# ishine/minimax-speech

Hardware: AMD Instinct MI355X
Metric: 24 kHz audio-seconds generated per wall-second per node (CosyVoice2-0.5B-shaped LM + flow + DAC-VAE, end to end) (higher is better)
Workload: dtype bf16

## Files before the change

include/mmx_hip.h:

```cpp
#ifndef MMX_HIP_H
#define MMX_HIP_H
#include <stdint.h>
#ifdef __cplusplus
extern "C" {
#endif

#ifndef __HIP__
typedef struct ihipStream_t* hipStream_t;
#endif

#define MMX_F32 0
#define MMX_BF16 1
#define MMX_X2 2
#define MMX_X3 3
#define MMX_X2W 0x12
#define MMX_X3W 0x13
#define MMX_H2 4
#define MMX_H2W 0x14

#define MMX_ACT_NONE 0
#define MMX_ACT_LRELU 1
#define MMX_ACT_GELU 2
#define MMX_ACT_SILU 3
#define MMX_ACT_MISH 4
#define MMX_ACT_TANH 5

int mmx_abi_version(void);

typedef struct MmxGemmParams {
    const void* A;
    const void* W;
    const float* bias;
    const float* residual;
    const float* rowmask;
    const float* alpha;
    float* out_f32;
    void* out_act;
    int64_t lda, ldw, ldr, ldo_f, ldo_a;
    int64_t a_bstride, w_bstride, r_bstride, rm_bstride, of_bstride, oa_bstride;
    int64_t row_off, row_lo, row_hi;
// ... 92 lines not shown

int mmx_decode_prep(const float* x, int64_t ldx, int B, int K, const float* gamma, float* h, int64_t ldh, void* xs,
                    float* ssq, int dtype, hipStream_t stream);
int mmx_skinny2(const void* xs, int B, int K, int N, const void* wp, const float* bias, const float* ssq_in, float eps,
                int epi, float* out, int64_t ldo, void* xs_out, const float* gamma_next, float* ssq_out,
                int tiles_per_wg, int ksplit, float* part, int64_t part_floats, int32_t* tickets, int dtype,
                hipStream_t stream);

int mmx_rope_kv_store(const float* qkv, int64_t ldqkv, int64_t qkv_bs, int B, int rows, int Hq, int Hkv, int D,
                      const float* inv_freq, const int32_t* pos, void* q_out, int64_t ldq, int64_t q_bs,
                      void* kc, void* vc, const int32_t* block_table, int max_pages, int page,
                      int dtype, hipStream_t stream);
int mmx_paged_attn(const void* q, int64_t ldq, int64_t q_bs, int B, int rows, int Hq, int Hkv, int D, float scale,
                   const int32_t* pos, const void* kc, const void* vc, const int32_t* block_table, int max_pages,
                   int page, void* out, int64_t ldo, int64_t o_bs, int dtype, hipStream_t stream);
#define MMX_DA_PACKED 1
#define MMX_DA_PER_HEAD 2
#define MMX_DA_SPLIT 4
#define MMX_DA_H2 8
#define MMX_DA_ONE_HEAD 16
int mmx_decode_attn(const float* qkv, int64_t ldqkv, int B, int Hq, int Hkv, int D, const float* inv_freq,
                    const float* rope_tab, const int32_t* pos, void* kc, void* vc, const int32_t* block_table, int max_pages, int page,
                    float scale, void* out, int64_t ldo, int dtype, int out_packed, hipStream_t stream);
int mmx_decode_attn_fin(const float* qkv, int64_t ldqkv, int B, int Hq, int Hkv, int D, const float* inv_freq,
                        const float* rope_tab, const int32_t* pos, const int32_t* finished, void* kc, void* vc,
                        const int32_t* block_table, int max_pages, int page, float scale, void* out, int64_t ldo, int dtype,
                        int out_packed, hipStream_t stream);
int mmx_swiglu(const float* gu, int64_t ldgu, int rows, int I, void* out, int64_t ldo, int dtype, hipStream_t stream);

int mmx_sample_step(const float* logits, int64_t ldl, int V, int B, int eos_id, int top_k, float top_p,
// ... 134 lines not shown
```

minimax-speech_amd/csrc/common.h:

```cpp
#pragma once
#include <hip/hip_runtime.h>
#include <stdint.h>
#include "../../include/mmx_hip.h"

#ifndef MMX_LAB
#define MMX_LAB 0
#endif
constexpr bool LAB = MMX_LAB != 0;

#define MMX_OK 0
#define MMX_EARG (-1)
#define MMX_CHECK_ARG(c) do { if (!(c)) return MMX_EARG; } while (0)
#define MMX_LAUNCH_CHECK() do { hipError_t e_ = hipGetLastError(); if (e_ != hipSuccess) return -(int)e_ - 1000; } while (0)

#define MMX_ACT_DTYPE(d) ((d) >= 2 ? 0 : (d))

#define MMX_LDS_OPT_IN(fn, bytes)                                                                                   \
    do {                                                                                                            \
        if ((bytes) > 64 * 1024) {                                                                                  \
            static bool done_[64] = {};                                                                             \
            int dev_ = 0;                                                                                           \
            if (hipGetDevice(&dev_) != hipSuccess || dev_ < 0 || dev_ >= 64) return MMX_EARG;                       \
            if (!done_[dev_]) {                                                                                     \
                hipError_t e_ = hipFuncSetAttribute((const void*)(fn), hipFuncAttributeMaxDynamicSharedMemorySize, 160 * 1024); \
// ... 55 lines not shown
#pragma unroll
    for (int o = 32; o > 0; o >>= 1) v += __shfl_xor(v, o, 64);
    return v;
}
__device__ __forceinline__ float wave_max(float v) {
#pragma unroll
    for (int o = 32; o > 0; o >>= 1) v = fmaxf(v, __shfl_xor(v, o, 64));
    return v;
}
__device__ __forceinline__ double wave_sum_f64(double v) {
#pragma unroll
    for (int o = 32; o > 0; o >>= 1) v += __shfl_xor(v, o, 64);
    return v;
}

enum { ACT_NONE = 0, ACT_LRELU = 1, ACT_GELU = 2, ACT_SILU = 3, ACT_MISH = 4, ACT_TANH = 5 };

__device__ __forceinline__ float erf_fast(float x) {
    const float ax = fabsf(x);
    const float t = __builtin_amdgcn_rcpf(1.0f + 0.3275911f * ax);
    float p = 1.061405429f;
    p = p * t - 1.453152027f;
    p = p * t + 1.421413741f;
    p = p * t - 0.284496736f;
    p = p * t + 0.254829592f;
    const float r = 1.0f - p * t * __expf(-ax * ax);
    return copysignf(r, x);
}

typedef float f32x2_t __attribute__((ext_vector_type(2)));
__device__ __forceinline__ f32x2_t gelu_fast2(f32x2_t v) {
// ... 90 lines not shown
```

minimax-speech_amd/csrc/gemm.hip:

```cpp
#include <algorithm>
#include "common.h"
#include "gemm.h"
#include <utility>

template <typename T> struct Frag;
template <> struct Frag<bf16_t> {
    static constexpr int CH = 8;
    static constexpr int LDS_ROW = 48;
};
template <> struct Frag<float> {
    static constexpr int CH = 4;
    static constexpr int LDS_ROW = 40;
};

template <typename T, typename TA, int NS, int BM, int BN, int WM, int WN, int NWP = 1>
__global__ __launch_bounds__(256) void gemm_win_kernel(GemmParams p) {
    constexpr int BK = 32;
    constexpr bool XS = NS > 1;
    static_assert(NWP == 1 || NWP == NS, "weight planes: as many as activation planes");
    static_assert(!XS || (sizeof(T) == 2 && sizeof(TA) == 4), "split build: bf16 weights, fp32 activations");
    static_assert(XS || sizeof(T) == sizeof(TA), "one storage type otherwise");
    constexpr int CH = Frag<T>::CH;
    constexpr int CPR = BK / CH;
    constexpr int CHA = 16 / sizeof(TA);
    constexpr int CPRA = BK / CHA;
    constexpr int LR = Frag<T>::LDS_ROW;
    constexpr int MF = BM / WM / 16, NF = BN / WN / 16;
    constexpr int A_CHUNKS = (BM * CPRA + 255) / 256, W_CHUNKS = (BN * CPR + 255) / 256;
    constexpr bool A_FULL = (BM * CPRA) % 256 == 0, W_FULL = (BN * CPR) % 256 == 0;
    constexpr bool PRECISE = sizeof(TA) == 4;
// ... 169 lines not shown
            load_tile(kt + STAGES, sc);
            __syncthreads();
            compute(decltype(sc)::value & 1);
        });
    }
    for_each_slot([&](auto sc) {
        const int kt = kt0 + decltype(sc)::value;
        if (kt < nk) {
            store_tile(decltype(sc)::value & 1, sc);
            __syncthreads();
            compute(decltype(sc)::value & 1);
        }
    });

    __syncthreads();
    constexpr int WNC = BN / WN;
    constexpr int CW = WNC / 4;
    constexpr int LDC = WNC + 4;
    float* Cs = reinterpret_cast<float*>(smem) + wave * 16 * LDC;
    float* outf = p.out_f32 ? p.out_f32 + (long)b * p.of_bstride : nullptr;
    TA* outa = p.out_act ? reinterpret_cast<TA*>(p.out_act) + (long)b * p.oa_bstride : nullptr;
    const float* res = p.residual ? p.residual + (long)b * p.r_bstride : nullptr;
    const float* rmask = p.rowmask ? p.rowmask + (long)b * p.rm_bstride : nullptr;
    constexpr int VA = 16 / sizeof(TA);
    const bool vec_f = outf && (p.ldo_f % 4 == 0) && (p.out_off % 4 == 0) && (p.of_bstride % 4 == 0) && ((uintptr_t)p.out_f32 % 16 == 0);
    const bool vec_a = outa && (p.ldo_a % VA == 0) && (p.out_off % VA == 0) && (p.oa_bstride % VA == 0) && ((uintptr_t)p.out_act % 16 == 0) && (CW % VA == 0);
    const bool vec_r = res && (p.ldr % 4 == 0) && (p.r_bstride % 4 == 0) && ((uintptr_t)p.residual % 16 == 0);
    const int erow = lane >> 2, ecol = (lane & 3) * CW;
    auto epilogue = [&](auto act_k, auto act2_k) {
    constexpr int ACT = decltype(act_k)::value, ACT2 = decltype(act2_k)::value;
// ... 92 lines not shown
    }
    };
    using std::integral_constant;
    switch (p.act) {
        case ACT_LRELU: epilogue(integral_constant<int, ACT_LRELU>{}, integral_constant<int, ACT_NONE>{}); break;
        case ACT_GELU: epilogue(integral_constant<int, ACT_GELU>{}, integral_constant<int, ACT_NONE>{}); break;
        case ACT_SILU: epilogue(integral_constant<int, ACT_SILU>{}, integral_constant<int, ACT_NONE>{}); break;
        case ACT_MISH: epilogue(integral_constant<int, ACT_MISH>{}, integral_constant<int, ACT_NONE>{}); break;
        case ACT_TANH: epilogue(integral_constant<int, ACT_TANH>{}, integral_constant<int, ACT_NONE>{}); break;
        default:
            if (p.act2 == ACT_MISH) epilogue(integral_constant<int, ACT_NONE>{}, integral_constant<int, ACT_MISH>{});
            else epilogue(integral_constant<int, ACT_NONE>{}, integral_constant<int, ACT_NONE>{});
    }
}

template <typename T, typename TA, int NS, int BM, int BN, int WM, int WN, int NWP = 1>
static int launch_cfg(const GemmParams& p, hipStream_t s) {
    dim3 grid((p.N + BN - 1) / BN, (p.M + BM - 1) / BM, p.batch);
    size_t lds = (size_t)2 * (NS * BM + NWP * BN) * Frag<T>::LDS_ROW * sizeof(T);
    const size_t lds_epi = (size_t)4 * 16 * (BN / WN + 4) * sizeof(float);
    if (lds_epi > lds) lds = lds_epi;
    MMX_LDS_OPT_IN((gemm_win_kernel<T, TA, NS, BM, BN, WM, WN, NWP>), lds);
    hipLaunchKernelGGL((gemm_win_kernel<T, TA, NS, BM, BN, WM, WN, NWP>), grid, dim3(256), lds, s, p);
    MMX_LAUNCH_CHECK();
    return MMX_OK;
}

template <typename T, typename TA, int NS, int NWP = 1>
static int launch_T(const GemmParams& p, hipStream_t s, int force_tile) {
    constexpr int CH = Frag<T>::CH;
    constexpr int CHA = 16 / sizeof(TA);
    MMX_CHECK_ARG(p.A && p.W && p.M > 0 && p.N > 0 && p.batch > 0 && p.ntaps >= 1);
    MMX_CHECK_ARG(p.cin % CH == 0 && p.lda % CHA == 0 && p.ldw % CH == 0);
    MMX_CHECK_ARG(p.a_bstride % CHA == 0 && p.w_bstride % CH == 0);
    MMX_CHECK_ARG(p.ldw % NWP == 0 && (p.ldw / NWP) % CH == 0 && p.ldw / NWP >= ((p.ntaps * p.cin + 31) / 32) * 32);
    MMX_CHECK_ARG(p.bias_mod > 0 && p.alpha_mod > 0 && p.row_stride >= 1);
    MMX_CHECK_ARG(((uintptr_t)p.A % 16) == 0 && ((uintptr_t)p.W % 16) == 0);
    MMX_CHECK_ARG(p.out_f32 || p.out_act);
    const long a_rows = std::min<long>(p.row_hi, (long)(p.M - 1) * p.row_stride + (long)(p.ntaps - 1) * p.dil + p.row_off + 1);
    MMX_CHECK_ARG((double)a_rows * (double)p.lda * sizeof(TA) < 2147483000.0 &&
                  (double)p.N * (double)p.ldw * sizeof(T) < 2147483000.0);
    MMX_CHECK_ARG(p.act2 == ACT_NONE || (p.act2 == ACT_MISH && p.act == ACT_NONE));
    auto blocks = [&](int bm, int bn) { return (long)((p.M + bm - 1) / bm) * ((p.N + bn - 1) / bn) * p.batch; };
    if constexpr (NWP > 1) {
        if (force_tile != 0 && force_tile != MMX_TILE_64x64 && force_tile != MMX_TILE_32x64) return MMX_EARG;
        if (force_tile != MMX_TILE_32x64 && (force_tile == MMX_TILE_64x64 || blocks(64, 64) >= 64 || p.M > 32))
            return launch_cfg<T, TA, NS, 64, 64, 2, 2, NWP>(p, s);
        return launch_cfg<T, TA, NS, 32, 64, 1, 4, NWP>(p, s);
    }
    switch (force_tile) {
        case 0: break;
        case MMX_TILE_128x128: return launch_cfg<T, TA, NS, 128, 128, 2, 2>(p, s);
        case MMX_TILE_128x64: return launch_cfg<T, TA, NS, 128, 64, 4, 1>(p, s);
        case MMX_TILE_64x64: return launch_cfg<T, TA, NS, 64, 64, 2, 2>(p, s);
        case MMX_TILE_32x64: return launch_cfg<T, TA, NS, 32, 64, 1, 4>(p, s);
        default: return MMX_EARG;
    }
// ... 21 lines not shown
```

minimax-speech_amd/csrc/llm.hip:

```cpp
#include "act_layout.h"
#include <type_traits>

template <typename T>
__global__ void pack_skinny_kernel(const T* __restrict__ w, long ldw, int N, int K, const float* __restrict__ kscale,
                                   int half, T* __restrict__ wp) {
    constexpr int E = sizeof(T) == 2 ? 8 : 4;
    constexpr int KB = E * 4;
    const long total = (long)((N + 15) / 16) * (K / KB) * 64 * E;
    for (long idx = (long)blockIdx.x * blockDim.x + threadIdx.x; idx < total; idx += (long)gridDim.x * blockDim.x) {
        int j = idx % E;
        long t = idx / E;
        int lane = t % 64;
        t /= 64;
        int kb = t % (K / KB);
        int tile = t / (K / KB);
        int col = lane & 15, g = lane >> 4;
        int row;
        if (half > 0) row = (tile & 1) * half + (tile >> 1) * 16 + col;
        else row = tile * 16 + col;
        int kk = kb * KB + g * E + j;
        float v = 0.f;
        if (row < N && (half == 0 || ((tile >> 1) * 16 + col) < half)) {
            v = Cvt<T>::to_f(w[(long)row * ldw + kk]);
            if (kscale) v *= kscale[kk];
// ... 418 lines not shown
    }
}
extern "C" int mmx_paged_attn(const void* q, int64_t ldq, int64_t q_bs, int B, int rows, int Hq, int Hkv, int D, float scale,
                              const int32_t* pos, const void* kc, const void* vc, const int32_t* block_table, int max_pages,
                              int page, void* out, int64_t ldo, int64_t o_bs, int dtype, hipStream_t stream) {
    dtype = MMX_ACT_DTYPE(dtype);
    MMX_CHECK_ARG(q && pos && kc && vc && block_table && out && B > 0 && rows > 0 && D == 64 && Hq % Hkv == 0 && page > 0);
    const size_t max_ctx = (size_t)max_pages * page;
    size_t lds = (64 + 8 + 4 * 64 + max_ctx) * 4;
    MMX_CHECK_ARG(lds <= 160 * 1024);
    return dispatch_dtype(dtype, [&](auto el) {
        using T = decltype(el);
        MMX_LDS_OPT_IN(paged_attn_kernel<T>, lds);
        hipLaunchKernelGGL(paged_attn_kernel<T>, dim3(Hq, rows, B), dim3(256), lds, stream, (const T*)q, ldq, q_bs, Hq, Hkv, scale, pos, (const T*)kc,
                           (const T*)vc, block_table, max_pages, page, (T*)out, ldo, o_bs);
        return launch_status();
    });
}

template <typename T>
struct Raw8 {
    uint4 a, b;
    __device__ __forceinline__ void load(const T* p) {
        a = *reinterpret_cast<const uint4*>(p);
        if constexpr (sizeof(T) == 4) b = *reinterpret_cast<const uint4*>(p + 4);
    }
    __device__ __forceinline__ void to_float(float o[8]) const {
        const unsigned w[4] = {a.x, a.y, a.z, a.w};
        if constexpr (sizeof(T) == 2) {
#pragma unroll
// ... 419 lines not shown
```

minimax-speech_amd/mmx/_lib.py:

```python
import ctypes as C
import os

import torch

F32, BF16 = 0, 1
X2, X3 = 2, 3
X2W, X3W = 0x12, 0x13
H2, H2W = 4, 0x14
DA_PACKED, DA_PER_HEAD, DA_SPLIT, DA_H2, DA_ONE_HEAD = 1, 2, 4, 8, 16
ACT = {"none": 0, "lrelu": 1, "gelu": 2, "silu": 3, "mish": 4, "tanh": 5}
TORCH_DT = {F32: torch.float32, BF16: torch.bfloat16, X2: torch.float32, X3: torch.float32, X2W: torch.float32, X3W: torch.float32}
WEIGHT_DT = {F32: torch.float32, BF16: torch.bfloat16, X2: torch.bfloat16, X3: torch.bfloat16, X2W: torch.bfloat16, X3W: torch.bfloat16}
ESIZE = {F32: 4, BF16: 2, X2: 4, X3: 4}
WPLANES = {X2W: 2, X3W: 3}
DTYPE_NAMES = {"f32": F32, "bf16": BF16, "x": X2, "x2": X2, "x3": X3}


def is_split(dtype):
    return dtype in (X2, X3, X2W, X3W)

_HERE = os.path.dirname(os.path.abspath(__file__))
LIB_PATH = os.environ.get("MMX_LIB") or os.path.join(os.path.dirname(_HERE), "lib", "libmmx_hip.so")

SYMBOLS = [
    "mmx_abi_version", "mmx_gemm_win", "mmx_gemm_win_tile", "mmx_rownorm", "mmx_groupnorm", "mmx_act_rows", "mmx_gather_rows", "mmx_copy2d", "mmx_est_pack",
    "mmx_sinusoidal_emb", "mmx_cfg_euler", "mmx_attn_dense", "mmx_attn_flash_bf16", "mmx_attn_flash_fp8", "mmx_attn_relpos_bf16", "mmx_attn_relpos_x", "mmx_attn_flash_x", "mmx_attn_flash_xs", "mmx_conv_cout1_tanh", "mmx_conv_cin1", "mmx_vae_sample", "mmx_resample_linear", "mmx_prefetch4", "mmx_mask_rows",
    "mmx_est_tail", "mmx_est_resnet", "mmx_dac_ru", "mmx_pack_skinny", "mmx_skinny_gemm", "mmx_skinny2", "mmx_decode_prep", "mmx_rope_kv_store", "mmx_paged_attn", "mmx_decode_attn", "mmx_decode_attn_fin", "mmx_swiglu", "mmx_sample_step",
    "mmx_sample_step_tab", "mmx_logmel", "mmx_pool_rows", "mmx_logmel_w", "mmx_s3_rope_fsmn", "mmx_fsq_encode", "mmx_resample_sinc", "mmx_kweight_blocks", "mmx_loudness_gate", "mmx_scale_rows",
    "mmx_spec_dist", "mmx_wave_sums", "mmx_gate_threshold", "mmx_gate_analyze", "mmx_gate_synthesize",
    "mmx_stoi_select", "mmx_stoi_bands", "mmx_stoi_score",
]


class GemmParams(C.Structure):
    _fields_ = [
        ("A", C.c_void_p), ("W", C.c_void_p), ("bias", C.c_void_p), ("residual", C.c_void_p),
        ("rowmask", C.c_void_p), ("alpha", C.c_void_p), ("out_f32", C.c_void_p), ("out_act", C.c_void_p),
        ("lda", C.c_int64), ("ldw", C.c_int64), ("ldr", C.c_int64), ("ldo_f", C.c_int64), ("ldo_a", C.c_int64),
        ("a_bstride", C.c_int64), ("w_bstride", C.c_int64), ("r_bstride", C.c_int64), ("rm_bstride", C.c_int64),
        ("of_bstride", C.c_int64), ("oa_bstride", C.c_int64),
        ("row_off", C.c_int64), ("row_lo", C.c_int64), ("row_hi", C.c_int64),
        ("out_off", C.c_int64), ("out_len", C.c_int64),
# ... 115 lines not shown
```

minimax-speech_amd/mmx/llm.py:

```python
import math
from typing import Dict, List, Optional

import torch

from . import ops
from ._lib import BF16, F32, H2, TORCH_DT, WEIGHT_DT, X3, X3W, is_split
from .flow import Graphed

ST_POS, ST_STEP, ST_NOUT, ST_FIN, ST_MINLEN, ST_MAXLEN, ST_SEQ, ST_ERR = range(8)


class PageAllocator:

    def __init__(self, n_pages: int):
        self.free_pages = list(range(n_pages - 1, -1, -1))
        self.n_pages = n_pages

    @property
    def n_free(self) -> int:
        return len(self.free_pages)

    def alloc(self, n: int) -> List[int]:
        if n > len(self.free_pages):
            raise RuntimeError(f"KV cache exhausted: {n} pages wanted, {len(self.free_pages)} free of {self.n_pages}")
# ... 26 lines not shown
            pk = lambda w, g=None, ih=0: ops.pack_skinny(c(w), dtype=dt, kscale=ks(g), interleave_half=ih)
        self.n_layers = len({k.split(".")[4] for k in sd if k.startswith(prefix + ".layers.")})
        self.H = sd[prefix + ".norm.weight"].shape[0]
        self.I = sd[prefix + ".layers.0.mlp.gate_proj.weight"].shape[0]
        self.layers, self.pf_layers = [], []
        for l in range(self.n_layers):
            p = f"{prefix}.layers.{l}"
            a = p + ".self_attn"
            wqkv = torch.cat([f(a + ".q_proj.weight"), f(a + ".k_proj.weight"), f(a + ".v_proj.weight")], 0)
            bqkv = torch.cat([f(a + ".q_proj.bias"), f(a + ".k_proj.bias"), f(a + ".v_proj.bias")], 0).contiguous()
            wgu = torch.cat([f(p + ".mlp.gate_proj.weight"), f(p + ".mlp.up_proj.weight")], 0)
            g1, g2 = f(p + ".input_layernorm.weight"), f(p + ".post_attention_layernorm.weight")
            if gemm_packs:
                self.pf_layers.append(dict(
                    wqkv=ops.pack_linear(c(wqkv), dt), wo=ops.pack_linear(c(f(a + ".o_proj.weight")), dt),
                    wgu=ops.pack_linear(c(wgu), dt), wdown=ops.pack_linear(c(f(p + ".mlp.down_proj.weight")), dt), g1=g1, g2=g2))
            self.layers.append(dict(wqkv=pk(wqkv, g1), bqkv=bqkv, wo=pk(f(a + ".o_proj.weight")), wgu=pk(wgu, g2, self.I),
                                    wdown=pk(f(p + ".mlp.down_proj.weight")), g1=g1, g2=g2))
            del wqkv, wgu
        self.norm_w = f(prefix + ".norm.weight")
        self.embed_tokens = f(prefix + ".embed_tokens.weight")
        if "llm_decoder.weight" in sd:
            self.wdec = pk(f("llm_decoder.weight"), self.norm_w)
            self.bdec = f("llm_decoder.bias")
            self.speech_emb = f("speech_embedding.weight")
            self.llm_emb = f("llm_embedding.weight")
        else:
            self.wdec = self.bdec = self.speech_emb = self.llm_emb = None
        self.inv_freq = (1.0 / (rope_theta ** (torch.arange(0, head_dim, 2, dtype=torch.int64).float() / head_dim))).to(self.dev)
        self.max_pages = (max_ctx + page - 1) // page
        self.max_out = self.max_pages * page
        ang = torch.arange(self.max_out, dtype=torch.float32)[:, None] * self.inv_freq.cpu()[None, :]
        self.rope_tab = torch.cat([ang.cos(), ang.sin()], dim=1).contiguous().to(self.dev)
        npages = max_batch * self.max_pages if kv_pages is None else int(kv_pages)
        self.trash_page = npages
        self.kc = torch.zeros(self.n_layers, npages + 1, kv_heads, page, head_dim, dtype=self.tdt, device=self.dev)
        self.vc = torch.zeros_like(self.kc)
        self.pages = PageAllocator(npages)


class LlmEngine:
    gqa_min_batch = 1 << 30
    use_v2 = True
    lm_planes = "f16x2"
    prefetch = 0
    skip_finished = True

    def __init__(self, sd: Dict[str, torch.Tensor], dtype=BF16, device="cuda", max_batch=1, max_ctx=2048, page=16,
                 heads=14, kv_heads=2, head_dim=64, rope_theta=1e6, eps=1e-6, speech_token_size=6561, use_graphs=True,
                 prefix="llm.model.model", share_from=None, kv_pages=None, wplanes=False, lm_planes=None, decode_on=None,
                 prompt_on=None):
        if share_from is not None:
            m, v2 = share_from.model, share_from.v2 if decode_on is None else decode_on == "planes"
            dtype, h2, wplanes, gemm_packs = m.dtype, m.h2, m.wplanes, bool(m.pf_layers)
        else:
            wplanes = dtype == X3 and ops.resolve_wplanes(wplanes, (v for k, v in sd.items() if v.dim() >= 2 and ("proj" in k or k == "llm_decoder.weight")))
            planes = lm_planes or self.lm_planes
            if planes not in ("f16x2", "bf16x3"):
                raise ValueError(f"lm_planes {planes!r}: 'f16x2' or 'bf16x3'")
            v2, gemm_packs = self.use_v2 if decode_on is None else decode_on == "planes", True
            h2 = dtype == X3 and planes == "f16x2" and v2
# ... 280 lines not shown
            for b, x in enumerate(lm_inputs):
                self._prefill(x, 0, b, head=True)
                self.state[ST_POS, b] = x.shape[0] - 1
        self._tail(B)
        self._fresh_decode_graph()

    def _prefill_batch(self, lm_inputs):
        B, H = self.B, self.H
        Ls = [int(x.shape[0]) for x in lm_inputs]
        Lm = max(Ls)
        R = B * Lm
        h = torch.zeros(B, Lm, H, device=self.dev)
        for b, x in enumerate(lm_inputs):
            h[b, :Ls[b]].copy_(x)
        h = h.reshape(R, H)
        self._gemm_layers(h, B, Lm, torch.zeros(B, dtype=torch.int32, device=self.dev), self.block_table)
        last = torch.tensor([b * Lm + Ls[b] - 1 for b in range(B)], dtype=torch.long, device=self.dev)
        hl = h.index_select(0, last)
        self.h[:B].copy_(hl)
        self.h_act[:B].copy_(hl)
        self.state[ST_POS].copy_(torch.tensor([L - 1 for L in Ls], dtype=torch.int32))

    def _gemm_layers(self, h, B, Lm, pos, block_table):
        m = self.model
        dt, H, I = m.dtype, m.H, m.I
        R = B * Lm
        a = torch.empty(R, H, dtype=m.tdt, device=self.dev)
        qkv = torch.empty(R, (m.Hq + 2 * m.Hkv) * m.D, device=self.dev)
        q = torch.empty(R, m.Hq * m.D, dtype=m.tdt, device=self.dev)
        att = torch.empty(R, m.Hq * m.D, dtype=m.tdt, device=self.dev)
        gu = torch.empty(R, 2 * I, device=self.dev)
        act = torch.empty(R, I, dtype=m.tdt, device=self.dev)
        for l, (w, ws) in enumerate(zip(m.pf_layers, m.layers)):
            ops.rownorm(h, w["g1"], None, m.eps, rows=R, C_=H, rms=True, out_act=a, dtype=dt)
            ops.linear(a, w["wqkv"], H, dtype=dt, bias=ws["bqkv"], out_f32=qkv)
            ops.rope_kv_store(qkv, m.inv_freq, pos, q, m.kc[l], m.vc[l], block_table, B=B, rows=Lm,
                              Hq=m.Hq, Hkv=m.Hkv, page=m.page, dtype=dt)
            ops.paged_attn(q, pos, m.kc[l], m.vc[l], block_table, att, B=B, rows=Lm, Hq=m.Hq,
                           Hkv=m.Hkv, page=m.page, dtype=dt)
            ops.linear(att, w["wo"], m.Hq * m.D, dtype=dt, residual=h, out_f32=h)
            ops.rownorm(h, w["g2"], None, m.eps, rows=R, C_=H, rms=True, out_act=a, dtype=dt)
            ops.linear(a, w["wgu"], H, dtype=dt, out_f32=gu)
            ops.swiglu(gu, act, rows=R, I=I, dtype=dt)
            ops.linear(act, w["wdown"], I, dtype=dt, residual=h, out_f32=h)

    def _prefill(self, x, pos0, slot, head=False, norm_out=None):
        m = self.model
        x = x.to(self.dev, torch.float32).contiguous()
        for c0 in range(0, x.shape[0], 64):
            hc, hca = self._prefill_chunk(x[c0:c0 + 64], pos0 + c0, slot)
            if norm_out is not None:
                ops.rownorm(hc, m.norm_w, None, m.eps, rows=hc.shape[0], C_=m.H, rms=True, out_f32=norm_out[c0:c0 + 64], dtype=F32)
        if head:
            self.h[slot].copy_(hc[-1])
            self.h_act[slot].copy_(hca[-1])

    def _prefill_chunk(self, xc, pos0, b):
        rows = xc.shape[0]
        if self.prompt_on == "gemm":
            hc = xc.to(self.dev, torch.float32).clone()
            self._gemm_layers(hc, 1, rows, torch.tensor([pos0], dtype=torch.int32, device=self.dev), self.block_table[b:b + 1].contiguous())
            return hc, hc.to(self.tdt)
        if not hasattr(self, "_pf"):
            self._pf = dict(h=torch.zeros(64, self.H, device=self.dev), ha=torch.zeros(64, self.H, dtype=self.tdt, device=self.dev),
                            pos=torch.zeros(1, dtype=torch.int32, device=self.dev),
                            bt=torch.zeros(1, self.max_pages, dtype=torch.int32, device=self.dev), graphs={})
        pf = self._pf
        pf["h"][:rows].copy_(xc)
        pf["ha"][:rows].copy_(xc)
        pf["pos"].fill_(pos0)
        pf["bt"].copy_(self.block_table[b:b + 1])
        if rows not in pf["graphs"]:
            pf["graphs"][rows] = Graphed(lambda r=rows: self._layers(pf["h"][:r], pf["ha"][:r], 1, r, pf["pos"], pf["bt"]), self.use_graphs)
        pf["graphs"][rows]()
        return pf["h"][:rows], pf["ha"][:rows]

# ... 183 lines not shown
```

minimax-speech_amd/mmx/ops.py:

```python
import ctypes as C
import math

import torch

from . import _lib as L
from ._lib import ACT, BF16, F32, check, i64, load, stream, _p


def round_up(x, m):
    return (x + m - 1) // m * m


class Planed(torch.Tensor):
    """A packed weight held as bf16 PLANES hi + [mid +] lo = w of an fp32 checkpoint's values (include/mmx_hip.h MMX_X2W / MMX_X3W).
    The type is the marker: gemm() / skinny2() switch to the weight-plane dtype code when they are handed one; views and row
    slices keep the type (torch's default __torch_function__)."""


def weight_planes(w: torch.Tensor, n: int):
    out, r = [], w.float()
    for _ in range(n):
        t = r.to(torch.bfloat16)
        out.append(t)
        r = r - t.float()
# ... 66 lines not shown
                      row_hi=(row_hi if row_hi is not None else (1 << 40)), out_off=out_off,
                      out_len=(out_len if out_len is not None else (1 << 62)), M=M, N=N, batch=batch,
                      ntaps=ntaps, cin=cin, dil=dil, bias_mod=(bias_mod or N), alpha_mod=(alpha_mod or N),
                      bias_per_row=int(bias_per_row), act=ACT[act], act2=ACT[act2], slope=slope, row_stride=row_stride)
    L.gemm_win(p, dtype, tile)


def linear(x, Wp, K, *, dtype, bias=None, act="none", act2="none", residual=None, rowmask=None, out_f32=None,
           out_act=None):
    N = Wp.shape[0]
    M = x.numel() // x.shape[-1]
    gemm(x, Wp, M, N, dtype=dtype, lda=x.shape[-1], cin=K, bias=bias, act=act, act2=act2,
         residual=residual, ldr=N, rowmask=rowmask, out_f32=out_f32, ldo_f=N, out_act=out_act, ldo_a=N)


def conv1d(x, Wp, *, T, Cin, k, dtype, dil=1, pad_left=0, batch=1, bias=None, act="none", slope=0.1, residual=None,
           rowmask=None, alpha=None, out_f32=None, out_act=None, T_out=None, act2="none", stride=1):
    Cout = Wp.shape[0]
    T_out = T if T_out is None else T_out
    gemm(x, Wp, T_out, Cout, dtype=dtype, lda=Cin, cin=Cin, ntaps=k, dil=dil, row_off=-pad_left, row_lo=0, row_hi=T, row_stride=stride,
         batch=batch, a_bstride=T * Cin, bias=bias, act=act, act2=act2, slope=slope,
         residual=residual, ldr=Cout, r_bstride=T_out * Cout, rowmask=rowmask, rm_bstride=T_out,
         alpha=alpha, out_f32=out_f32, ldo_f=Cout, of_bstride=T_out * Cout,
         out_act=out_act, ldo_a=Cout, oa_bstride=T_out * Cout)


def convtranspose1d(x, Wp, *, T, Cin, Cout, stride, dtype, batch=1, bias=None, alpha=None, out_f32=None, out_act=None):
    s = stride
    pad = math.ceil(s / 2)
    gemm(x, Wp, T + 1, s * Cout, dtype=dtype, lda=Cin, cin=Cin, ntaps=2, dil=1, row_off=-1, row_lo=0, row_hi=T,
# ... 300 lines not shown
    ldqkv = (Hq + 2 * Hkv) * 64 if ldqkv is None else ldqkv
    ldq = Hq * 64 if ldq is None else ldq
    check(load().mmx_rope_kv_store(_p(qkv), i64(ldqkv), i64(rows * ldqkv if qkv_bs is None else qkv_bs), B, rows, Hq, Hkv, 64,
                                   _p(inv_freq), _p(pos), _p(q_out), i64(ldq), i64(rows * ldq if q_bs is None else q_bs), _p(kc), _p(vc),
                                   _p(block_table), block_table.shape[1], page, dtype, stream()), "mmx_rope_kv_store")


def paged_attn(q, pos, kc, vc, block_table, out, *, B, rows, Hq, Hkv, page, dtype, ldq=None, q_bs=None, ldo=None, o_bs=None):
    ldq = Hq * 64 if ldq is None else ldq
    ldo = Hq * 64 if ldo is None else ldo
    check(load().mmx_paged_attn(_p(q), i64(ldq), i64(rows * ldq if q_bs is None else q_bs), B, rows, Hq, Hkv, 64, C.c_float(0.125),
                                _p(pos), _p(kc), _p(vc), _p(block_table), block_table.shape[1], page, _p(out),
                                i64(ldo), i64(rows * ldo if o_bs is None else o_bs), dtype, stream()), "mmx_paged_attn")


def decode_attn_bits(out_packed=False, per_head=False, out_split=False, one_head=False):
    return ((L.DA_PACKED if out_packed else 0) | (L.DA_PER_HEAD if per_head else 0) | (L.DA_ONE_HEAD if one_head else 0) |
            (L.DA_H2 if out_split == "f16" else L.DA_SPLIT if out_split else 0))


def decode_attn(qkv, inv_freq, pos, kc, vc, block_table, out, *, B, Hq, Hkv, page, dtype, rope_tab=None, out_packed=False,
                per_head=False, out_split=False, one_head=False, ldqkv=None, ldo=None, finished=None):
    assert finished is None or (finished.dtype == torch.int32 and finished.numel() >= B and finished.stride(-1) == 1)
    check(load().mmx_decode_attn_fin(_p(qkv), i64((Hq + 2 * Hkv) * 64 if ldqkv is None else ldqkv), B, Hq, Hkv, 64, _p(inv_freq), _p(rope_tab),
                                     _p(pos), _p(finished), _p(kc), _p(vc), _p(block_table), block_table.shape[1], page, C.c_float(0.125), _p(out),
                                     i64(Hq * 64 if ldo is None else ldo), dtype, decode_attn_bits(out_packed, per_head, out_split, one_head), stream()), "mmx_decode_attn_fin")


def swiglu(gu, out, *, rows, I, dtype, ldgu=None, ldo=None):
    check(load().mmx_swiglu(_p(gu), i64(ldgu or 2 * I), rows, I, _p(out), i64(ldo or I), dtype, stream()), "mmx_swiglu")
# ... 31 lines not shown
```

Measured before the change: 567.7.

## Fuse SwiGLU into gate/up GEMM epilogue and add tiled prompt attention kernel

The prompt-phase LM layers now compute gate/up with a GEMM whose epilogue applies SiLU(gate)*up directly and writes the activation. Gate and up weight rows are interleaved in blocks of 16 so each wave holds matching fragments. This removes the fp32 gu buffer and the separate swiglu kernel. A new prompt attention kernel loads the whole short KV context (up to 256) into LDS per KV head and processes 8 query rows per block with all 7 grouped Q heads, replacing paged_attn when shapes fit. The costs are a forced 64x64 tile for the GLU GEMM, heavy LDS use, and a kernel that only covers small prompts.

Result: no change. 570.3 (median of 6 runs) (+0.5%).

```diff
diff --git a/include/mmx_hip.h b/include/mmx_hip.h
--- a/include/mmx_hip.h
+++ b/include/mmx_hip.h
@@ -24,6 +24,7 @@
 #define MMX_ACT_SILU 3
 #define MMX_ACT_MISH 4
 #define MMX_ACT_TANH 5
+#define MMX_ACT_SWIGLU 6
 
 int mmx_abi_version(void);
 
@@ -146,6 +147,9 @@
 int mmx_paged_attn(const void* q, int64_t ldq, int64_t q_bs, int B, int rows, int Hq, int Hkv, int D, float scale,
                    const int32_t* pos, const void* kc, const void* vc, const int32_t* block_table, int max_pages,
                    int page, void* out, int64_t ldo, int64_t o_bs, int dtype, hipStream_t stream);
+int mmx_prompt_attn(const void* q, int64_t ldq, int64_t q_bs, int B, int rows, int Hq, int Hkv, int D, float scale,
+                    const int32_t* pos, const void* kc, const void* vc, const int32_t* block_table, int max_pages,
+                    int page, void* out, int64_t ldo, int64_t o_bs, int ctx_max, int dtype, hipStream_t stream);
 #define MMX_DA_PACKED 1
 #define MMX_DA_PER_HEAD 2
 #define MMX_DA_SPLIT 4
diff --git a/minimax-speech_amd/csrc/common.h b/minimax-speech_amd/csrc/common.h
--- a/minimax-speech_amd/csrc/common.h
+++ b/minimax-speech_amd/csrc/common.h
@@ -93,7 +93,8 @@
     return v;
 }
 
-enum { ACT_NONE = 0, ACT_LRELU = 1, ACT_GELU = 2, ACT_SILU = 3, ACT_MISH = 4, ACT_TANH = 5 };
+enum { ACT_NONE = 0, ACT_LRELU = 1, ACT_GELU = 2, ACT_SILU = 3, ACT_MISH = 4, ACT_TANH = 5,
+       ACT_SWIGLU = 6 };
 
 __device__ __forceinline__ float erf_fast(float x) {
     const float ax = fabsf(x);
diff --git a/minimax-speech_amd/csrc/gemm.hip b/minimax-speech_amd/csrc/gemm.hip
--- a/minimax-speech_amd/csrc/gemm.hip
+++ b/minimax-speech_amd/csrc/gemm.hip
@@ -13,7 +13,7 @@
     static constexpr int LDS_ROW = 40;
 };
 
-template <typename T, typename TA, int NS, int BM, int BN, int WM, int WN, int NWP = 1>
+template <typename T, typename TA, int NS, int BM, int BN, int WM, int WN, int NWP = 1, bool GLU = false>
 __global__ __launch_bounds__(256) void gemm_win_kernel(GemmParams p) {
     constexpr int BK = 32;
     constexpr bool XS = NS > 1;
@@ -213,6 +213,58 @@
     });
 
     __syncthreads();
+    if constexpr (GLU) {
+        static_assert(NF % 2 == 0 && (BN / WN / 8) % 4 == 0, "gate and up fragments come in pairs; a lane stores whole groups of 4 columns");
+        constexpr int WNO = BN / WN / 2;
+        constexpr int CWO = WNO / 4;
+        constexpr int LDO = WNO + 4;
+        float* Cs = reinterpret_cast<float*>(smem) + wave * 16 * LDO;
+        TA* outa = reinterpret_cast<TA*>(p.out_act) + (long)b * p.oa_bstride;
+        const int NO = p.N / 2;
+        const bool vec = (p.ldo_a % (16 / sizeof(TA)) == 0) && (p.oa_bstride % (16 / sizeof(TA)) == 0) && ((uintptr_t)p.out_act % 16 == 0);
+        const int erow = lane >> 2, ecol = (lane & 3) * CWO;
+#pragma unroll
+        for (int i = 0; i < MF; ++i) {
+#pragma unroll
+            for (int jj = 0; jj < NF / 2; ++jj)
+#pragma unroll
+                for (int r = 0; r < 4; ++r) {
+                    const float gt = acc[i][2 * jj][r], u = acc[i][2 * jj + 1][r];
+                    const float s = gt / (1.f + expf(-gt));
+                    Cs[(4 * g + r) * LDO + jj * 16 + l16] = s * u;
+                }
+            __builtin_amdgcn_fence(__ATOMIC_RELEASE, "wavefront");
+            __builtin_amdgcn_wave_barrier();
+            float v[CWO];
+#pragma unroll
+            for (int c = 0; c < CWO; c += 4) {
+                float4_t t4 = *reinterpret_cast<const float4_t*>(Cs + erow * LDO + ecol + c);
+                v[c] = t4[0]; v[c + 1] = t4[1]; v[c + 2] = t4[2]; v[c + 3] = t4[3];
+            }
+            __builtin_amdgcn_wave_barrier();
+            const int m = m0 + wm * (BM / WM) + i * 16 + erow;
+            const int nb = n0 / 2 + wn * WNO + ecol;
+            if (m >= p.M || nb >= NO) continue;
+            TA* o = outa + (long)m * p.ldo_a + nb;
+            if (vec) {
+#pragma unroll
+                for (int c = 0; c < CWO; c += 4) {
+                    if constexpr (sizeof(TA) == 2) {
+                        uint2 pk;
+                        pk.x = (unsigned)Cvt<TA>::from_f(v[c]) | ((unsigned)Cvt<TA>::from_f(v[c + 1]) << 16);
+                        pk.y = (unsigned)Cvt<TA>::from_f(v[c + 2]) | ((unsigned)Cvt<TA>::from_f(v[c + 3]) << 16);
+                        *reinterpret_cast<uint2*>(o + c) = pk;
+                    } else {
+                        *reinterpret_cast<float4_t*>(o + c) = float4_t{v[c], v[c + 1], v[c + 2], v[c + 3]};
+                    }
+                }
+            } else {
+#pragma unroll
+                for (int c = 0; c < CWO; ++c) o[c] = Cvt<TA>::from_f(v[c]);
+            }
+        }
+        return;
+    }
     constexpr int WNC = BN / WN;
     constexpr int CW = WNC / 4;
     constexpr int LDC = WNC + 4;
@@ -335,14 +387,14 @@
     }
 }
 
-template <typename T, typename TA, int NS, int BM, int BN, int WM, int WN, int NWP = 1>
+template <typename T, typename TA, int NS, int BM, int BN, int WM, int WN, int NWP = 1, bool GLU = false>
 static int launch_cfg(const GemmParams& p, hipStream_t s) {
     dim3 grid((p.N + BN - 1) / BN, (p.M + BM - 1) / BM, p.batch);
     size_t lds = (size_t)2 * (NS * BM + NWP * BN) * Frag<T>::LDS_ROW * sizeof(T);
     const size_t lds_epi = (size_t)4 * 16 * (BN / WN + 4) * sizeof(float);
     if (lds_epi > lds) lds = lds_epi;
-    MMX_LDS_OPT_IN((gemm_win_kernel<T, TA, NS, BM, BN, WM, WN, NWP>), lds);
-    hipLaunchKernelGGL((gemm_win_kernel<T, TA, NS, BM, BN, WM, WN, NWP>), grid, dim3(256), lds, s, p);
+    MMX_LDS_OPT_IN((gemm_win_kernel<T, TA, NS, BM, BN, WM, WN, NWP, GLU>), lds);
+    hipLaunchKernelGGL((gemm_win_kernel<T, TA, NS, BM, BN, WM, WN, NWP, GLU>), grid, dim3(256), lds, s, p);
     MMX_LAUNCH_CHECK();
     return MMX_OK;
 }
@@ -362,6 +414,11 @@
     MMX_CHECK_ARG((double)a_rows * (double)p.lda * sizeof(TA) < 2147483000.0 &&
                   (double)p.N * (double)p.ldw * sizeof(T) < 2147483000.0);
     MMX_CHECK_ARG(p.act2 == ACT_NONE || (p.act2 == ACT_MISH && p.act == ACT_NONE));
+    if (p.act == ACT_SWIGLU) {
+        MMX_CHECK_ARG(p.N % 32 == 0 && p.out_act && !p.out_f32 && !p.bias && !p.residual && !p.rowmask && !p.alpha && p.out_off == 0);
+        MMX_CHECK_ARG(force_tile == 0 || force_tile == MMX_TILE_64x64);
+        return launch_cfg<T, TA, NS, 64, 64, 2, 2, NWP, true>(p, s);
+    }
     auto blocks = [&](int bm, int bn) { return (long)((p.M + bm - 1) / bm) * ((p.N + bn - 1) / bn) * p.batch; };
     if constexpr (NWP > 1) {
         if (force_tile != 0 && force_tile != MMX_TILE_64x64 && force_tile != MMX_TILE_32x64) return MMX_EARG;
diff --git a/minimax-speech_amd/csrc/llm.hip b/minimax-speech_amd/csrc/llm.hip
--- a/minimax-speech_amd/csrc/llm.hip
+++ b/minimax-speech_amd/csrc/llm.hip
@@ -456,6 +456,139 @@
         MMX_LDS_OPT_IN(paged_attn_kernel<T>, lds);
         hipLaunchKernelGGL(paged_attn_kernel<T>, dim3(Hq, rows, B), dim3(256), lds, stream, (const T*)q, ldq, q_bs, Hq, Hkv, scale, pos, (const T*)kc,
                            (const T*)vc, block_table, max_pages, page, (T*)out, ldo, o_bs);
+        return launch_status();
+    });
+}
+
+constexpr int PA_R = 8, PA_G = 7, PA_KP = 68, PA_CTX = 256, PA_ROWS = 64;
+constexpr int PA_DFMA = 54;
+__device__ __forceinline__ float mul_rn(float a, float b) {
+#pragma clang fp contract(off)
+    return a * b;
+}
+__device__ __forceinline__ float add_rn(float a, float b) {
+#pragma clang fp contract(off)
+    return a + b;
+}
+template <typename T>
+__device__ __forceinline__ float4 load4f(const T* p) {
+    if constexpr (sizeof(T) == 4) {
+        return *reinterpret_cast<const float4*>(p);
+    } else {
+        const uint2 w = *reinterpret_cast<const uint2*>(p);
+        return make_float4(__uint_as_float(w.x << 16), __uint_as_float(w.x & 0xffff0000u), __uint_as_float(w.y << 16),
+                           __uint_as_float(w.y & 0xffff0000u));
+    }
+}
+template <typename T>
+__global__ __launch_bounds__(256) void prompt_attn_kernel(
+    const T* __restrict__ q, long ldq, long q_bs, int rows, int Hkv, float scale, const int32_t* __restrict__ pos,
+    const T* __restrict__ kc, const T* __restrict__ vc, const int32_t* __restrict__ block_table, int max_pages,
+    int page, T* __restrict__ out, long ldo, long o_bs, int ctx_max) {
+    constexpr int D = 64, G = PA_G, NG = PA_CTX / 64;
+    extern __shared__ __attribute__((aligned(16))) char smem[];
+    float* Ks = reinterpret_cast<float*>(smem);
+    float* Vs = Ks + (long)ctx_max * PA_KP;
+    const int tid = threadIdx.x, lane = tid & 63, wave = __builtin_amdgcn_readfirstlane(tid >> 6);
+    const int hk = blockIdx.x, t0 = blockIdx.y * PA_R, b = blockIdx.z;
+    const int p0 = pos[b];
+    const int t_end = t0 + PA_R < rows ? t0 + PA_R : rows;
+    const int nk = p0 + t_end;
+    if (p0 < 0 || nk > ctx_max) return;
+    const int32_t* bt = block_table + (long)b * max_pages;
+    for (int i = tid; i < nk * (D / 4); i += 256) {
+        const int j = i >> 4, c = (i & 15) * 4;
+        const long at = (((long)bt[j / page] * Hkv + hk) * page + j % page) * D + c;
+        *reinterpret_cast<float4*>(Ks + j * PA_KP + c) = load4f(kc + at);
+        *reinterpret_cast<float4*>(Vs + j * D + c) = load4f(vc + at);
+    }
+    __syncthreads();
+    for (int t = t0 + wave; t < t_end; t += 4) {
+        const int ctx = p0 + t + 1;
+        const T* __restrict__ qr = q + (long)b * q_bs + (long)t * ldq + (long)hk * G * D;
+        float e[NG][G];
+        float wm[NG][G], ws[NG][G];
+#pragma unroll
+        for (int g = 0; g < NG; ++g) {
+#pragma unroll
+            for (int h = 0; h < G; ++h) { e[g][h] = 0.f; wm[g][h] = -INFINITY; ws[g][h] = 0.f; }
+            if (g * 64 < ctx) {
+                const int j = g * 64 + lane;
+                const float* kp = Ks + (j < ctx ? j : ctx - 1) * PA_KP;
+                float s[G];
+#pragma unroll
+                for (int h = 0; h < G; ++h) s[h] = 0.f;
+#pragma unroll
+                for (int d = 0; d < D; d += 4) {
+                    const float4 k4 = *reinterpret_cast<const float4*>(kp + d);
+                    const float kd[4] = {k4.x, k4.y, k4.z, k4.w};
+#pragma unroll
+                    for (int h = 0; h < G; ++h)
+#pragma unroll
+                        for (int c = 0; c < 4; ++c) {
+                            const float qd = Cvt<T>::to_f(qr[h * D + d + c]);
+                            s[h] = d + c < PA_DFMA ? __builtin_fmaf(qd, kd[c], s[h]) : add_rn(s[h], mul_rn(qd, kd[c]));
+                        }
+                }
+#pragma unroll
+                for (int h = 0; h < G; ++h) {
+                    e[g][h] = mul_rn(s[h], scale);
+                    wm[g][h] = wave_max(j < ctx ? e[g][h] : -INFINITY);
+                }
+            }
+        }
+        float l[G];
+#pragma unroll
+        for (int h = 0; h < G; ++h) {
+            const float mx = fmaxf(fmaxf(wm[0][h], wm[1][h]), fmaxf(wm[2][h], wm[3][h]));
+#pragma unroll
+            for (int g = 0; g < NG; ++g)
+                if (g * 64 < ctx) {
+                    e[g][h] = g * 64 + lane < ctx ? expf(add_rn(e[g][h], -mx)) : 0.f;
+                    ws[g][h] = wave_sum(e[g][h]);
+                }
+            l[h] = add_rn(add_rn(add_rn(ws[0][h], ws[1][h]), ws[2][h]), ws[3][h]);
+        }
+        float acc[4][G];
+#pragma unroll
+        for (int w = 0; w < 4; ++w)
+#pragma unroll
+            for (int h = 0; h < G; ++h) acc[w][h] = 0.f;
+#pragma unroll
+        for (int g = 0; g < NG; ++g) {
+            if (g * 64 < ctx) {
+                const int jn = ctx - g * 64 < 64 ? ctx - g * 64 : 64;
+                for (int j0 = 0; j0 < jn; j0 += 4) {
+#pragma unroll
+                    for (int w = 0; w < 4; ++w) {
+                        if (j0 + w < jn) {
+                            const float v = Vs[(g * 64 + j0 + w) * D + lane];
+#pragma unroll
+                            for (int h = 0; h < G; ++h)
+                                acc[w][h] = __builtin_fmaf(__builtin_bit_cast(float, __builtin_amdgcn_readlane(__builtin_bit_cast(int, e[g][h]), j0 + w)), v, acc[w][h]);
+                        }
+                    }
+                }
+            }
+        }
+        T* o = out + (long)b * o_bs + (long)t * ldo + (long)hk * G * D + lane;
+#pragma unroll
+        for (int h = 0; h < G; ++h) o[h * D] = Cvt<T>::from_f(add_rn(add_rn(acc[0][h], acc[1][h]), add_rn(acc[2][h], acc[3][h])) / l[h]);
+    }
+}
+extern "C" int mmx_prompt_attn(const void* q, int64_t ldq, int64_t q_bs, int B, int rows, int Hq, int Hkv, int D, float scale,
+                               const int32_t* pos, const void* kc, const void* vc, const int32_t* block_table, int max_pages,
+                               int page, void* out, int64_t ldo, int64_t o_bs, int ctx_max, int dtype, hipStream_t stream) {
+    dtype = MMX_ACT_DTYPE(dtype);
+    MMX_CHECK_ARG(q && pos && kc && vc && block_table && out && B > 0 && rows > 0 && D == 64 && Hkv > 0 && Hq == PA_G * Hkv && page > 0);
+    MMX_CHECK_ARG(rows <= PA_ROWS && ctx_max >= rows && ctx_max <= PA_CTX && (long)ctx_max <= (long)max_pages * page);
+    MMX_CHECK_ARG(((uintptr_t)kc % 16) == 0 && ((uintptr_t)vc % 16) == 0);
+    const size_t lds = (size_t)ctx_max * (PA_KP + 64) * 4;
+    return dispatch_dtype(dtype, [&](auto el) {
+        using T = decltype(el);
+        MMX_LDS_OPT_IN(prompt_attn_kernel<T>, lds);
+        hipLaunchKernelGGL(prompt_attn_kernel<T>, dim3(Hkv, (rows + PA_R - 1) / PA_R, B), dim3(256), lds, stream, (const T*)q, ldq, q_bs, rows, Hkv,
+                           scale, pos, (const T*)kc, (const T*)vc, block_table, max_pages, page, (T*)out, ldo, o_bs, ctx_max);
         return launch_status();
     });
 }
diff --git a/minimax-speech_amd/mmx/_lib.py b/minimax-speech_amd/mmx/_lib.py
--- a/minimax-speech_amd/mmx/_lib.py
+++ b/minimax-speech_amd/mmx/_lib.py
@@ -25,7 +25,7 @@
 SYMBOLS = [
     "mmx_abi_version", "mmx_gemm_win", "mmx_gemm_win_tile", "mmx_rownorm", "mmx_groupnorm", "mmx_act_rows", "mmx_gather_rows", "mmx_copy2d", "mmx_est_pack",
     "mmx_sinusoidal_emb", "mmx_cfg_euler", "mmx_attn_dense", "mmx_attn_flash_bf16", "mmx_attn_flash_fp8", "mmx_attn_relpos_bf16", "mmx_attn_relpos_x", "mmx_attn_flash_x", "mmx_attn_flash_xs", "mmx_conv_cout1_tanh", "mmx_conv_cin1", "mmx_vae_sample", "mmx_resample_linear", "mmx_prefetch4", "mmx_mask_rows",
-    "mmx_est_tail", "mmx_est_resnet", "mmx_dac_ru", "mmx_pack_skinny", "mmx_skinny_gemm", "mmx_skinny2", "mmx_decode_prep", "mmx_rope_kv_store", "mmx_paged_attn", "mmx_decode_attn", "mmx_decode_attn_fin", "mmx_swiglu", "mmx_sample_step",
+    "mmx_est_tail", "mmx_est_resnet", "mmx_dac_ru", "mmx_pack_skinny", "mmx_skinny_gemm", "mmx_skinny2", "mmx_decode_prep", "mmx_rope_kv_store", "mmx_paged_attn", "mmx_prompt_attn", "mmx_decode_attn", "mmx_decode_attn_fin", "mmx_swiglu", "mmx_sample_step",
     "mmx_sample_step_tab", "mmx_logmel", "mmx_pool_rows", "mmx_logmel_w", "mmx_s3_rope_fsmn", "mmx_fsq_encode", "mmx_resample_sinc", "mmx_kweight_blocks", "mmx_loudness_gate", "mmx_scale_rows",
     "mmx_spec_dist", "mmx_wave_sums", "mmx_gate_threshold", "mmx_gate_analyze", "mmx_gate_synthesize",
     "mmx_stoi_select", "mmx_stoi_bands", "mmx_stoi_score",
diff --git a/minimax-speech_amd/mmx/llm.py b/minimax-speech_amd/mmx/llm.py
--- a/minimax-speech_amd/mmx/llm.py
+++ b/minimax-speech_amd/mmx/llm.py
@@ -1,3 +1,4 @@
+import functools
 import math
 from typing import Dict, List, Optional
 
@@ -64,7 +65,7 @@
             if gemm_packs:
                 self.pf_layers.append(dict(
                     wqkv=ops.pack_linear(c(wqkv), dt), wo=ops.pack_linear(c(f(a + ".o_proj.weight")), dt),
-                    wgu=ops.pack_linear(c(wgu), dt), wdown=ops.pack_linear(c(f(p + ".mlp.down_proj.weight")), dt), g1=g1, g2=g2))
+                    wgu=ops.pack_glu(c(wgu), dt), wdown=ops.pack_linear(c(f(p + ".mlp.down_proj.weight")), dt), g1=g1, g2=g2))
             self.layers.append(dict(wqkv=pk(wqkv, g1), bqkv=bqkv, wo=pk(f(a + ".o_proj.weight")), wgu=pk(wgu, g2, self.I),
                                     wdown=pk(f(p + ".mlp.down_proj.weight")), g1=g1, g2=g2))
             del wqkv, wgu
@@ -95,6 +96,7 @@
     lm_planes = "f16x2"
     prefetch = 0
     skip_finished = True
+    prompt_attn = "tiles"
 
     def __init__(self, sd: Dict[str, torch.Tensor], dtype=BF16, device="cuda", max_batch=1, max_ctx=2048, page=16,
                  heads=14, kv_heads=2, head_dim=64, rope_theta=1e6, eps=1e-6, speech_token_size=6561, use_graphs=True,
@@ -405,34 +407,35 @@
         for b, x in enumerate(lm_inputs):
             h[b, :Ls[b]].copy_(x)
         h = h.reshape(R, H)
-        self._gemm_layers(h, B, Lm, torch.zeros(B, dtype=torch.int32, device=self.dev), self.block_table)
+        self._gemm_layers(h, B, Lm, torch.zeros(B, dtype=torch.int32, device=self.dev), self.block_table, ctx_max=Lm)
         last = torch.tensor([b * Lm + Ls[b] - 1 for b in range(B)], dtype=torch.long, device=self.dev)
         hl = h.index_select(0, last)
         self.h[:B].copy_(hl)
         self.h_act[:B].copy_(hl)
         self.state[ST_POS].copy_(torch.tensor([L - 1 for L in Ls], dtype=torch.int32))
 
-    def _gemm_layers(self, h, B, Lm, pos, block_table):
+    def _gemm_layers(self, h, B, Lm, pos, block_table, ctx_max):
         m = self.model
         dt, H, I = m.dtype, m.H, m.I
         R = B * Lm
+        if self.prompt_attn not in ("tiles", "paged"):
+            raise ValueError(f"prompt_attn {self.prompt_attn!r}: 'tiles' or 'paged'")
+        tiles = self.prompt_attn == "tiles" and ops.prompt_attn_ok(Lm, ctx_max, m.Hq, m.Hkv)
+        attn = functools.partial(ops.prompt_attn, ctx_max=ctx_max) if tiles else ops.paged_attn
         a = torch.empty(R, H, dtype=m.tdt, device=self.dev)
         qkv = torch.empty(R, (m.Hq + 2 * m.Hkv) * m.D, device=self.dev)
         q = torch.empty(R, m.Hq * m.D, dtype=m.tdt, device=self.dev)
         att = torch.empty(R, m.Hq * m.D, dtype=m.tdt, device=self.dev)
-        gu = torch.empty(R, 2 * I, device=self.dev)
         act = torch.empty(R, I, dtype=m.tdt, device=self.dev)
         for l, (w, ws) in enumerate(zip(m.pf_layers, m.layers)):
             ops.rownorm(h, w["g1"], None, m.eps, rows=R, C_=H, rms=True, out_act=a, dtype=dt)
             ops.linear(a, w["wqkv"], H, dtype=dt, bias=ws["bqkv"], out_f32=qkv)
             ops.rope_kv_store(qkv, m.inv_freq, pos, q, m.kc[l], m.vc[l], block_table, B=B, rows=Lm,
                               Hq=m.Hq, Hkv=m.Hkv, page=m.page, dtype=dt)
-            ops.paged_attn(q, pos, m.kc[l], m.vc[l], block_table, att, B=B, rows=Lm, Hq=m.Hq,
-                           Hkv=m.Hkv, page=m.page, dtype=dt)
+            attn(q, pos, m.kc[l], m.vc[l], block_table, att, B=B, rows=Lm, Hq=m.Hq, Hkv=m.Hkv, page=m.page, dtype=dt)
             ops.linear(att, w["wo"], m.Hq * m.D, dtype=dt, residual=h, out_f32=h)
             ops.rownorm(h, w["g2"], None, m.eps, rows=R, C_=H, rms=True, out_act=a, dtype=dt)
-            ops.linear(a, w["wgu"], H, dtype=dt, out_f32=gu)
-            ops.swiglu(gu, act, rows=R, I=I, dtype=dt)
+            ops.linear_glu(a, w["wgu"], H, dtype=dt, out_act=act)
             ops.linear(act, w["wdown"], I, dtype=dt, residual=h, out_f32=h)
 
     def _prefill(self, x, pos0, slot, head=False, norm_out=None):
@@ -450,7 +453,8 @@
         rows = xc.shape[0]
         if self.prompt_on == "gemm":
             hc = xc.to(self.dev, torch.float32).clone()
-            self._gemm_layers(hc, 1, rows, torch.tensor([pos0], dtype=torch.int32, device=self.dev), self.block_table[b:b + 1].contiguous())
+            self._gemm_layers(hc, 1, rows, torch.tensor([pos0], dtype=torch.int32, device=self.dev), self.block_table[b:b + 1].contiguous(),
+                              ctx_max=pos0 + rows)
             return hc, hc.to(self.tdt)
         if not hasattr(self, "_pf"):
             self._pf = dict(h=torch.zeros(64, self.H, device=self.dev), ha=torch.zeros(64, self.H, dtype=self.tdt, device=self.dev),
diff --git a/minimax-speech_amd/mmx/ops.py b/minimax-speech_amd/mmx/ops.py
--- a/minimax-speech_amd/mmx/ops.py
+++ b/minimax-speech_amd/mmx/ops.py
@@ -104,6 +104,29 @@
          residual=residual, ldr=N, rowmask=rowmask, out_f32=out_f32, ldo_f=N, out_act=out_act, ldo_a=N)
 
 
+GLU_BLOCK = 16
+ACT_SWIGLU = 6
+
+
+def pack_glu(wgu: torch.Tensor, dtype) -> torch.Tensor:
+    I2, K = wgu.shape
+    assert I2 % (2 * GLU_BLOCK) == 0, "gate/up width must be a multiple of 16"
+    return pack_linear(wgu.reshape(2, I2 // 2 // GLU_BLOCK, GLU_BLOCK, K).transpose(0, 1).reshape(I2, K), dtype)
+
+
+def linear_glu(x, Wp, K, *, dtype, out_act):
+    N = Wp.shape[0]
+    M = x.numel() // x.shape[-1]
+    ldw = Wp.shape[-1]
+    if isinstance(Wp, Planed):
+        dtype = {L.X2: L.X2W, L.X3: L.X3W, L.X2W: L.X2W, L.X3W: L.X3W}[dtype]
+    elif dtype in L.WPLANES:
+        raise L.MmxError("a weight-plane dtype needs a Planed weight (ops.pack_glu with X2W / X3W)")
+    p = L.gemm_params(A=x, W=Wp, out_act=out_act, lda=x.shape[-1], ldw=ldw, ldo_a=N // 2, M=M, N=N, cin=K, bias_mod=N, alpha_mod=N,
+                      row_hi=1 << 40, act=ACT_SWIGLU)
+    L.gemm_win(p, dtype)
+
+
 def conv1d(x, Wp, *, T, Cin, k, dtype, dil=1, pad_left=0, batch=1, bias=None, act="none", slope=0.1, residual=None,
            rowmask=None, alpha=None, out_f32=None, out_act=None, T_out=None, act2="none", stride=1):
     Cout = Wp.shape[0]
@@ -434,6 +457,21 @@
                                 i64(ldo), i64(rows * ldo if o_bs is None else o_bs), dtype, stream()), "mmx_paged_attn")
 
 
+PROMPT_ATTN_CTX, PROMPT_ATTN_ROWS, PROMPT_ATTN_GROUP = 256, 64, 7
+
+
+def prompt_attn_ok(rows, ctx_max, Hq, Hkv):
+    return rows <= PROMPT_ATTN_ROWS and ctx_max <= PROMPT_ATTN_CTX and Hq == PROMPT_ATTN_GROUP * Hkv
+
+
+def prompt_attn(q, pos, kc, vc, block_table, out, *, B, rows, Hq, Hkv, page, dtype, ctx_max, ldq=None, q_bs=None, ldo=None, o_bs=None):
+    ldq = Hq * 64 if ldq is None else ldq
+    ldo = Hq * 64 if ldo is None else ldo
+    check(load().mmx_prompt_attn(_p(q), i64(ldq), i64(rows * ldq if q_bs is None else q_bs), B, rows, Hq, Hkv, 64, C.c_float(0.125),
+                                 _p(pos), _p(kc), _p(vc), _p(block_table), block_table.shape[1], page, _p(out),
+                                 i64(ldo), i64(rows * ldo if o_bs is None else o_bs), int(ctx_max), dtype, stream()), "mmx_prompt_attn")
+
+
 def decode_attn_bits(out_packed=False, per_head=False, out_split=False, one_head=False):
     return ((L.DA_PACKED if out_packed else 0) | (L.DA_PER_HEAD if per_head else 0) | (L.DA_ONE_HEAD if one_head else 0) |
             (L.DA_H2 if out_split == "f16" else L.DA_SPLIT if out_split else 0))
```
